# thimabru1010/ResUnet-a_mltsk_keras

Hardware: AMD Instinct MI355X
Metric: training patches/sec (256×256, 6-ch, bs=8/GPU) at 1/2/4/8 MI355X (higher is better)
Workload: dtype bf16; 1 GPU; cfg3: ResUnet-a d6 multitask (seg+bound+dist+color) Tanimoto-dual, 256x256x6, 6 classes, Adam, full train step (fwd+loss+bwd+allreduce+update); global_batch=8, per_gpu_batch=8, parallelism=dp1

## Files before the change

### include/rua_hip.h

```cpp
#ifndef RUA_HIP_H
#define RUA_HIP_H
#include <stdint.h>
#ifdef __cplusplus
extern "C" {
#endif

#define RUA_F32 0
#define RUA_BF16 1
#define RUA_MAX_SEG 6
#define RUA_MAX_BRANCH 4
#define RUA_MAX_WGRAD_BATCH 32
#define RUA_MAX_WGRAD_GROUP 8

#define RUA_OK 0
#define RUA_ERR_ARG (-1)
#define RUA_ERR_LAUNCH (-2)

int rua_version(void);
const char* rua_last_error(void);
int rua_device_info(int* cu_count, int* lds_bytes, char* arch, int arch_len);

typedef struct rua_conv_seg {
  const void* x;
  const void* w;
// ... 91 lines not shown
  const int32_t* overwrite_dev;
} rua_wgrad_desc;
typedef struct rua_wgrad_pending {
  int32_t kind;
  int32_t parts;
  int64_t n;
  const float* partials;
  float* dw;
  int32_t CC;
  int32_t blocks;
  int32_t block_begin, pad;
  const int32_t* overwrite_dev;
} rua_wgrad_pending;
int rua_wgrad_plan(const rua_wgrad_desc* d, rua_wgrad_pending* out);
int rua_wgrad_reduce_batch(const rua_wgrad_pending* items_dev, int n_items, int total_blocks, void* stream);
int rua_conv_wgrad(const rua_wgrad_desc* d, void* stream);
int rua_conv_wgrad_group(const rua_wgrad_desc* d, int n, void* stream);
int rua_wgrad_group_last_grids(void);
int rua_wgrad_group_plan(const rua_wgrad_desc* d, int n, rua_wgrad_pending* out);
int64_t rua_wgrad_workspace_bytes(const rua_wgrad_desc* d);
int rua_wgrad_kind(const rua_wgrad_desc* d);
int rua_wgrad_img_kind(const rua_wgrad_desc* d);

typedef struct rua_wprep_item { int64_t src_off, dst_off; int32_t taps, Cout, C, pad; } rua_wprep_item;
int rua_weight_prep(const float* master, void* w_fwd, void* w_dgrad, const rua_wprep_item* items_dev,
                    int n_items, int max_elems, int dtype, void* stream);
int rua_weight_prep_dgrad(const void* w_fwd, void* w_dgrad, const rua_wprep_item* items_dev, int n_items, int max_elems, const int32_t* blockmap_dev,
                          int n_blocks, int dtype, void* stream);
int rua_wprep_blocks(int taps, int Cout, int C);

// ... 152 lines not shown
int64_t rua_lovasz_workspace_bytes(int64_t M, int C);
int rua_lovasz_grad(const float* p, const float* y, const uint8_t* void_mask, int64_t M, int C, int all_classes, float loss_weight,
                    void* workspace, int64_t workspace_bytes, double* loss_out, float* dp, uint32_t* order_out,
                    rua_lovasz_result* result_dev, void* stream);
int rua_lovasz_dz(int act, const float* p, const float* dp, const float* scale_dev, int64_t M, int C, float* dz, void* stream);

int rua_lr_step(double* state, float* lr_out, int adam, double beta1, double beta2, void* stream);
int rua_adam_step(float* theta, float* g, float* m, float* v, int64_t n, float lr_t, const float* lr_t_dev, float beta1, float beta2,
                  float eps, float grad_scale, int zero_grad, void* stream);
int rua_sgd_step(float* theta, float* g, float* vel, int64_t n, float lr, const float* lr_dev, float momentum, float grad_scale,
                 int zero_grad, void* stream);
int rua_adam_step_w(float* theta, float* g, float* m, float* v, int64_t n, float lr_t, const float* lr_t_dev, float beta1, float beta2,
                    float eps, float grad_scale, int zero_grad, void* wcopy_bf16, void* stream);
int rua_sgd_step_w(float* theta, float* g, float* vel, int64_t n, float lr, const float* lr_dev, float momentum, float grad_scale,
                   int zero_grad, void* wcopy_bf16, void* stream);

#define RUA_OPT_CHUNK 8192
typedef struct rua_opt_chunk { int64_t off; int32_t len; int32_t var; } rua_opt_chunk;
typedef struct rua_opt_var { int32_t chunk_begin, chunk_end, decay, pad; } rua_opt_var;
#define RUA_CLIP_NONE 0
#define RUA_CLIP_GLOBAL_NORM 1
#define RUA_CLIP_NORM 2
#define RUA_CLIP_VALUE 3
int rua_grad_sumsq(const float* g, const rua_opt_chunk* chunks, int n_chunks, double* partials, void* stream);
int rua_clip_finish(const double* partials, int n_chunks, const rua_opt_var* vars, int n_vars, int mode, double c, double grad_scale,
                    int skip_nonfinite, double* var_sumsq, float* coef, int32_t* flag, double* report, void* stream);
int rua_adam_step_seg(float* theta, float* g, float* m, float* v, const rua_opt_chunk* chunks, int n_chunks, const rua_opt_var* vars,
                      const float* coef, const int32_t* flag, const float* lr_dev, const double* lr_state, float beta1, float beta2, float eps,
                      float grad_scale, float clipvalue, double weight_decay, int zero_grad, void* wcopy_bf16, void* stream);
int rua_sgd_step_seg(float* theta, float* g, float* vel, const rua_opt_chunk* chunks, int n_chunks, const rua_opt_var* vars,
// ... 127 lines not shown
```

### resunet_a_mltsk_keras_amd/_lib.py

```python
from __future__ import annotations

import ctypes as C
import os

HERE = os.path.dirname(os.path.abspath(__file__))
LIB_PATH = os.environ.get("RUA_LIB_PATH") or os.path.join(HERE, "librua_hip.so")

RUA_F32, RUA_BF16 = 0, 1
RUA_MAX_SEG, RUA_MAX_BRANCH, RUA_MAX_WGRAD_GROUP, RUA_MAX_WGRAD_BATCH = 6, 4, 8, 32
LOSS_TANIMOTO, LOSS_WCE, LOSS_CE_LOGITS, LOSS_BCE_LOGITS, LOSS_MSE, LOSS_FOCAL_CE, LOSS_FOCAL_BCE = 0, 1, 2, 3, 4, 5, 6
LOSS_LOVASZ, RUA_LOVASZ_MAX_C = 7, 16
ACT_NONE, ACT_SOFTMAX, ACT_SIGMOID = 0, 1, 2

vp, i32, i64, f32, f64 = C.c_void_p, C.c_int32, C.c_int64, C.c_float, C.c_double


class ConvSeg(C.Structure):
    _fields_ = [("x", vp), ("w", vp), ("C", i32), ("Hs", i32), ("Ws", i32), ("up_shift", i32), ("dil", i32), ("taps", i32)]


class ConvDesc(C.Structure):
    _fields_ = [("seg", ConvSeg * RUA_MAX_SEG), ("nseg", i32), ("N", i32), ("H", i32), ("W", i32), ("Cout", i32),
                ("stride", i32), ("dtype", i32), ("bias", vp), ("aux", vp), ("aux_mode", i32), ("mscale", vp),
                ("mshift", vp), ("out_relu", i32), ("accumulate", i32), ("y", vp), ("out_stride", i32), ("OH", i32),
# ... 107 lines not shown
    "rua_wgrad_group_last_grids": ([], i32),
    "rua_wgrad_group_plan": ([C.POINTER(WgradDesc), i32, C.POINTER(WgradPending)], i32),
    "rua_profile_mid_event": ([vp], None),
    "rua_profile_mid_event_fired": ([], i32),
    "rua_prof_event_create": ([], vp),
    "rua_prof_event_record": ([vp, vp], i32),
    "rua_prof_event_elapsed_us": ([vp, vp, C.POINTER(f64)], i32),
    "rua_prof_event_destroy": ([vp], None),
    "rua_graph_kernel_nodes": ([vp, C.POINTER(i32), C.POINTER(i32)], i32),
    "rua_conv_workspace_bytes": ([C.POINTER(ConvDesc)], i64),
    "rua_conv_wgrad": ([C.POINTER(WgradDesc), vp], i32),
    "rua_wgrad_workspace_bytes": ([C.POINTER(WgradDesc)], i64),
    "rua_wgrad_kind": ([C.POINTER(WgradDesc)], i32),
    "rua_wgrad_img_kind": ([C.POINTER(WgradDesc)], i32),
    "rua_wgrad_plan": ([C.POINTER(WgradDesc), C.POINTER(WgradPending)], i32),
    "rua_wgrad_reduce_batch": ([vp, i32, i32, vp], i32),
    "rua_weight_prep": ([vp, vp, vp, vp, i32, i32, i32, vp], i32),
    "rua_weight_prep_dgrad": ([vp, vp, vp, i32, i32, vp, i32, i32, vp], i32),
    "rua_wprep_blocks": ([i32, i32, i32], i32),
    "rua_stem_fwd": ([vp, vp, vp, vp, i64, i32, i32, i32, vp], i32),
    "rua_stem_fwd_stats": ([vp, vp, vp, vp, i64, i32, i32, i32, vp, i32, vp], i32),
    "rua_stem_bwd": ([vp, vp, vp, vp, i64, i32, i32, i32, vp], i32),
    "rua_stem_fwd_pack": ([vp, vp, vp, vp, i64, i32, i32, i32, vp, i32, vp, vp], i32),
    "rua_stem_bwd_fold": ([vp, vp, vp, i32, i32, vp], i32),
    "rua_head_fwd": ([vp, vp, vp, vp, vp, i64, i32, i32, i32, i32, vp], i32),
    "rua_head_fwd_loss": ([vp, vp, vp, vp, vp, vp, vp, vp, i32, i64, i32, i32, i32, i32, vp], i32),
    "rua_head_fwd_loss_rep": ([vp, vp, vp, vp, vp, vp, vp, i32, vp, i32, i64, i32, i32, i32, i32, vp], i32),
    "rua_head_bwd": ([vp, vp, vp, vp, i32, vp, vp, vp, i64, i64, i32, i32, i32, i32, vp], i32),
    "rua_head_bwd_sums": ([vp, vp, vp, vp, i32, vp, vp, vp, vp, i64, i64, i32, i32, i32, i32, vp], i32),
    "rua_col_stats": ([vp, i64, i32, vp, i32, i32, vp], i32),
# ... 28 lines not shown
    "rua_fill_zero": ([vp, i64, vp], i32),
    "rua_tanimoto_sums": ([vp, vp, i32, i64, i32, vp, vp], i32),
    "rua_tanimoto_finalize": ([vp, i32, i64, i32, f32, vp, vp, vp, vp], i32),
    "rua_tanimoto_finalize_rep": ([vp, i32, i32, i64, i32, f32, vp, vp, vp, vp], i32),
    "rua_tanimoto_finalize_multi": ([vp, i32, vp], i32),
    "rua_head_dz_multi": ([vp, i32, vp], i32),
    "rua_tanimoto_ratio": ([vp, i32, i32, vp, vp, vp], i32),
    "rua_pixel_loss": ([i32, vp, vp, vp, vp, i64, i32, vp, vp, vp], i32),
    "rua_head_dz": ([i32, i32, vp, vp, vp, vp, f32, i32, i64, i32, vp, vp], i32),
    "rua_seg_metrics": ([vp, vp, i64, i32, vp, vp], i32),
    "rua_lr_step": ([vp, vp, i32, f64, f64, vp], i32),
    "rua_adam_step": ([vp, vp, vp, vp, i64, f32, vp, f32, f32, f32, f32, i32, vp], i32),
    "rua_sgd_step": ([vp, vp, vp, i64, f32, vp, f32, f32, i32, vp], i32),
    "rua_adam_step_w": ([vp, vp, vp, vp, i64, f32, vp, f32, f32, f32, f32, i32, vp, vp], i32),
    "rua_sgd_step_w": ([vp, vp, vp, i64, f32, vp, f32, f32, i32, vp, vp], i32),
    "rua_grad_sumsq": ([vp, vp, i32, vp, vp], i32),
    "rua_clip_finish": ([vp, i32, vp, i32, i32, f64, f64, i32, vp, vp, vp, vp, vp], i32),
    "rua_adam_step_seg": ([vp, vp, vp, vp, vp, i32, vp, vp, vp, vp, vp, f32, f32, f32, f32, f32, f64, i32, vp, vp], i32),
    "rua_sgd_step_seg": ([vp, vp, vp, vp, i32, vp, vp, vp, vp, vp, f32, f32, f32, f64, i32, vp, vp], i32),
    "rua_state_copy": ([vp, vp, i64, vp, vp], i32),
    "rua_lr_schedule_step": ([vp, vp, LrSchedule, i32, f64, f64, vp], i32),
    "rua_ema_step": ([vp, vp, vp, i64, f32, vp, i32, vp, vp], i32),
    "rua_accum_gate": ([vp, i32, vp, vp], i32),
    "rua_accum_step": ([vp, vp, i64, i32, vp, vp], i32),
    "rua_lr_step_gated": ([vp, vp, i32, f64, f64, vp, vp], i32),
    "rua_lr_schedule_step_gated": ([vp, vp, LrSchedule, i32, f64, f64, vp, vp], i32),
    "rua_grad_sumsq_gated": ([vp, vp, i32, vp, vp, vp], i32),
    "rua_clip_finish_gated": ([vp, i32, vp, i32, i32, f64, f64, i32, vp, vp, vp, vp, vp, vp], i32),
    "rua_lamb_moments": ([vp, vp, vp, vp, vp, i32, vp, vp, vp, vp, f32, f32, f32, f32, f32, f64, vp, vp, vp], i32),
    "rua_lamb_finish": ([vp, vp, i32, vp, i32, vp, vp, vp, vp, vp], i32),
# ... 114 lines not shown
```

### resunet_a_mltsk_keras_amd/csrc/conv_wgrad.hip

```cpp
#include "common.h"

struct WgK {
  const unsigned char* a; const unsigned char* dy; float* dw;
  int C, Hs, Ws, Cout, H, W, N, stride, dil, taps;
  long long M; int pix_per_block, ntc, nti, ksplit;
  int wshift, hshift;
  float* slabs;
  const int* overwrite;
};

template <typename T>
__device__ __forceinline__ void wgrad_kernel_body(const WgK& p, int b) {
  constexpr int VEC = ET<T>::VEC, ES = sizeof(T);
  constexpr int TP = 64;
  constexpr int PPR = 64 / VEC;
  constexpr int ROWB = (ES == 2) ? 192 : 260;
  constexpr int PASS = TP * PPR / 256;
  __shared__ __attribute__((aligned(16))) unsigned char sD[TP * ROWB];
  __shared__ __attribute__((aligned(16))) unsigned char sX[TP * ROWB];

  const int ks = b % p.ksplit; b /= p.ksplit;
  const int ti = b % p.nti; b /= p.nti;
  const int tc = b % p.ntc; b /= p.ntc;
  const int tap = b;
// ... 1848 lines not shown
  return RUA_OK;
}
static int wgrad_issue_alone(const WgLaunch& L, hipStream_t st) {
  const WgLaunch* one = &L;
  const int rc = wgrad_issue(&one, 1, st);
  if (rc != RUA_OK || L.defer || !L.pending.kind) return rc;
  rua_record_mid_event(st);
  return wgrad_reduce(L.pending, st);
}

extern "C" int rua_wgrad_plan(const rua_wgrad_desc* d, rua_wgrad_pending* out) {
  RUA_CHECK_ARG(d && out, "rua_wgrad_plan: null pointer");
  WgLaunch L;
  return wgrad_plan_record(d, 0, &L, out);
}
extern "C" int rua_conv_wgrad(const rua_wgrad_desc* d, void* stream) {
  WgLaunch L;
  const int rc = wgrad_plan_one(d, 0, &L);
  return rc != RUA_OK ? rc : wgrad_issue_alone(L, (hipStream_t)stream);
}

static thread_local int g_wg_group_last_grids = 0;
extern "C" int rua_wgrad_group_last_grids(void) { return g_wg_group_last_grids; }

constexpr int WG_BATCH_MAX_MEMBERS = 4 * RUA_MAX_WGRAD_BATCH;
static bool wgrad_batch_ok(const rua_wgrad_desc* d, int n) {
  if (!(g_tune.wgrad_group & 1) || n > WG_BATCH_MAX_MEMBERS) return false;
  for (int i = 0; i < n; ++i) {
    if (!d[i].a || !d[i].dy || !d[i].dw || d[i].dtype != RUA_BF16 || !d[i].batch || d[i].in_scale) return false;
    if (d[i].C <= 0 || d[i].Cout <= 0 || d[i].C % 8 || d[i].Cout % 8 || (d[i].taps != 1 && d[i].taps != 9)) return false;
// ... 152 lines not shown
```

### resunet_a_mltsk_keras_amd/csrc/loss_optim.hip

```cpp
#include "common.h"

__device__ __forceinline__ void block_atomic_add(double* dst, float v, float* sh , int slot) {
  v = wave_sum(v);
  const int lane = threadIdx.x & 63, wid = threadIdx.x >> 6;
  if (lane == 0) sh[slot * 4 + wid] = v;
  __syncthreads();
  if (threadIdx.x == 0) unsafeAtomicAdd(dst, (double)sh[slot * 4 + 0] + (double)sh[slot * 4 + 1] + (double)sh[slot * 4 + 2] + (double)sh[slot * 4 + 3]);
  __syncthreads();
}

template <bool VM>
__global__ __launch_bounds__(256) void tanimoto_sums_kernel(const float* __restrict__ p, const float* __restrict__ y, long long HW, int C,
                                                            int pix_per_block, double* sums, const uint8_t* __restrict__ vm) {
  __shared__ float sh[4 * 48];
  const int n = blockIdx.y;
  float acc[8][6];
#pragma unroll
  for (int c = 0; c < 8; ++c)
#pragma unroll
    for (int k = 0; k < 6; ++k) acc[c][k] = 0.f;
  long long i = (long long)blockIdx.x * pix_per_block + threadIdx.x;
  long long iend = (long long)(blockIdx.x + 1) * pix_per_block; if (iend > HW) iend = HW;
  for (; i < iend; i += 256) {
    if constexpr (VM) { if (vm[(size_t)n * HW + i]) continue; }
// ... 848 lines not shown
  }
}
template <bool WC>
__global__ __launch_bounds__(256) void sgd_kernel(float* __restrict__ th, float* __restrict__ g, float* __restrict__ vel,
                                                  long long n, float lr, const float* __restrict__ lr_dev, float mu, float gs, int zero, bf16_t* __restrict__ wcopy) {
  if (lr_dev) lr = lr_dev[0];
  for (long long i = (long long)blockIdx.x * 256 + threadIdx.x; i < n; i += (long long)gridDim.x * 256) {
    const float vv = mu * vel[i] - lr * g[i] * gs;
    vel[i] = vv;
    const float tt = th[i] + vv;
    th[i] = tt;
    if (zero) g[i] = 0.f;
    if constexpr (WC) wcopy[i] = (bf16_t)tt;
  }
}
__global__ void lr_step_kernel(double* state, float* lr_out, int adam, double beta1, double beta2, const int32_t* hold) {
  if (blockIdx.x == 0 && threadIdx.x == 0 && !(hold != nullptr && hold[0] != 0)) {
    const double t = state[0] + 1.0;
    state[0] = t;
    double lr = state[1];
    if (adam) lr = lr * sqrt(1.0 - pow(beta2, t)) / (1.0 - pow(beta1, t));
    lr_out[0] = (float)lr;
  }
}
extern "C" int rua_lr_step(double* state, float* lr_out, int adam, double beta1, double beta2, void* stream) {
  RUA_CHECK_ARG(state && lr_out, "rua_lr_step: null pointer");
  hipLaunchKernelGGL(lr_step_kernel, dim3(1), dim3(64), 0, (hipStream_t)stream, state, lr_out, adam, beta1, beta2, (const int32_t*)nullptr);
  RUA_LAUNCH_CHECK("rua_lr_step");
  return RUA_OK;
}
// ... 17 lines not shown
                             float eps, float grad_scale, int zero_grad, void* stream) {
  return rua_adam_step_w(theta, g, m, v, n, lr_t, lr_t_dev, beta1, beta2, eps, grad_scale, zero_grad, nullptr, stream);
}
extern "C" int rua_sgd_step_w(float* theta, float* g, float* vel, int64_t n, float lr, const float* lr_dev, float momentum, float grad_scale,
                              int zero_grad, void* wcopy_bf16, void* stream) {
  RUA_CHECK_ARG(theta && g && vel && n > 0, "rua_sgd_step: bad arguments");
  int64_t gr = (n + 255) / 256; if (gr > 4096) gr = 4096;
  if (wcopy_bf16) hipLaunchKernelGGL((sgd_kernel<true>), dim3((int)gr), dim3(256), 0, (hipStream_t)stream, theta, g, vel, (long long)n, lr, lr_dev, momentum, grad_scale, zero_grad, (bf16_t*)wcopy_bf16);
  else hipLaunchKernelGGL((sgd_kernel<false>), dim3((int)gr), dim3(256), 0, (hipStream_t)stream, theta, g, vel, (long long)n, lr, lr_dev, momentum, grad_scale, zero_grad, (bf16_t*)nullptr);
  RUA_LAUNCH_CHECK("rua_sgd_step");
  return RUA_OK;
}
extern "C" int rua_sgd_step(float* theta, float* g, float* vel, int64_t n, float lr, const float* lr_dev, float momentum, float grad_scale,
                            int zero_grad, void* stream) {
  return rua_sgd_step_w(theta, g, vel, n, lr, lr_dev, momentum, grad_scale, zero_grad, nullptr, stream);
}

__device__ __forceinline__ double wave_sum_f64(double v) {
#pragma unroll
  for (int o = 32; o > 0; o >>= 1) v += __shfl_xor(v, o, 64);
  return v;
}
__global__ __launch_bounds__(256) void grad_sumsq_kernel(const float* __restrict__ g, const rua_opt_chunk* __restrict__ chunks, double* __restrict__ partials,
                                                         const int32_t* __restrict__ hold) {
  __shared__ double sh[4];
  if (hold != nullptr && hold[0] != 0) return;
  const rua_opt_chunk ck = chunks[blockIdx.x];
  const float* gp = g + ck.off;
  const int n4 = ck.len >> 2;
  double acc = 0.0;
// ... 405 lines not shown
```

### resunet_a_mltsk_keras_amd/engine.py

```python
from __future__ import annotations

import contextlib
import ctypes as C
import math
import os
from dataclasses import dataclass, field
from typing import Dict, List, Optional, Tuple

import numpy as np
import torch

from . import _lib as L
from . import accum as AC
from . import clip as CL
from . import lamb as LB
from . import losses as LS
from . import schedules as SC
from .wgrad_queue import WgradQueue, WSpec
from .scenes import (BLEND_MODES, MAP_HEADS, AffineSceneBatch, SceneBatch, blend_table, check_blend_budget, check_photo_table, check_radius,
                     check_scales, check_tolerance, check_views, instance_params, instance_scores, scale_table, sieve_params, sweep_params,
                     view_rows)

BN_EPS, BN_MOMENTUM, KERAS_EPS = 1e-3, 0.99, 1e-7
HEADS = ["seg", "bound", "dist", "color"]
# ... 215 lines not shown
        return self.N * self.H * self.W


def stats_replicas(blocks: int) -> int:
    r = 1
    while r < 32 and r * 8 < blocks:
        r *= 2
    return r


def conv_stats_replicas(blocks: int) -> int:
    r = 1
    while r < 32 and r * 64 < blocks:
        r *= 2
    return r


class Stat:
    __slots__ = ("ptr", "R")

    def __init__(self, ptr, R):
        self.ptr, self.R = ptr, R


class _Dummy:

    def __init__(self, n=0):
        self._n = n

    def data_ptr(self):
# ... 845 lines not shown
                self.wq.one(Bp, WSpec(x, dy, lay["segs"][0]["off"], 1, 1, 9))
                gx, acc = self.gacc(x, masked=x.relu_out)
                sx = None
                if x.bias_offs and x.relu_out and not acc and not self.dry and self.e.bn_dx_bias:
                    sx = self.stat(x.C, (x.M + 127) // 128)
                self.dgrad(Bp, dy, self.Wd(lay["segs"][0]["dst"]), x.C, 1, 9, gx, acc, mask=(x, None, None) if x.relu_out else None, stats2=sx)
                if sx is not None:
                    self.stats_to_grads(Bp, sx, x.C, x.bias_offs)
                    x.bias_done = True
            self.back_steps.append(back)
        return y

    def head(self, x: Ten, cout: int, act: int, hname: str, name=None, lay=None):
        F, tr = self.fwd, self.training
        lay = lay if lay is not None else self.Lconv([x.C], cout, 1, name=name, mfma=False)
        z = self.new(x.N, x.H, x.W, cout, f32=True)
        p = self.new(x.N, x.H, x.W, cout, f32=True)
        y = self.new(x.N, x.H, x.W, cout, f32=True)
        h = dict(name=hname, x=x, z=z, p=p, y=y, lay=lay, act=act, C=cout, slot=len(self.heads))
        sp = self.e.loss
        tani = sp is not None and sp.kind.get(hname) == L.LOSS_TANIMOTO
        if sp is not None and not self.dry and self.e.fuse_head_loss and (tani or hname == "seg"):
            if tani:
                h["sums_rep"] = SUMS_REPLICAS
                h["sums"] = self.salloc((SUMS_REPLICAS + 1) * x.N * cout * 6)
            if hname == "seg":
                h["metrics_done"] = True
            head_args = (x.ptr, self.P(lay["segs"][0]["off"]), self.P(lay["bias"]), z.ptr, p.ptr, y.ptr, h.get("sums"),
                         h.get("sums_rep", 1), self.e.scalars_ptr + 8 * 8 if hname == "seg" else None, x.N, x.H * x.W, x.C, cout, act, self.dt)
            if self.void_ptr is not None:
                F.add("rua_head_fwd_loss_void", *head_args, self.void_ptr)
            else:
                F.add("rua_head_fwd_loss_rep", *head_args)
        else:
            F.add("rua_head_fwd", x.ptr, self.P(lay["segs"][0]["off"]), self.P(lay["bias"]), z.ptr, p.ptr, x.M, x.C, cout, act, self.dt)
        self.heads.append(h)
        return h
# ... 311 lines not shown
class Engine:

    def __init__(self, cfg: ModelConfig, dtype: str = "bf16", device: Optional[torch.device] = None, seed: int = 0,
                 split_k: bool = True, _layout_only: bool = False):
        assert dtype in ("bf16", "f32")
        self.cfg = cfg
        self.dt = L.RUA_BF16 if dtype == "bf16" else L.RUA_F32
        self.dtype = dtype
        self.esize = 2 if dtype == "bf16" else 4
        if cfg.width % 32 != 0:
            raise ValueError(f"width={cfg.width}: the first-stage width must be a multiple of 32 (PSP branches are width/4 "
                             "channels and the MFMA epilogue stores 8-channel pieces)")
        self.dev = None
        self.fuse_bn = os.environ.get("RUA_FUSE_BN", "1") != "0"
        self.fuse_head_loss = os.environ.get("RUA_FUSE_HEAD_LOSS", "1") != "0"
        self.bn_out_stats = os.environ.get("RUA_BN_OUT_STATS", "1") != "0"
        self.bn_dx_bias = os.environ.get("RUA_BN_DX_BIAS", "1") != "0"
        self.pool_pyramid = os.environ.get("RUA_POOL_PYRAMID", "1") != "0"
        self.fold_bn = os.environ.get("RUA_FOLD_BN", "1") != "0"
        self.defer_reduce = os.environ.get("RUA_DEFER_REDUCE", "1") != "0"
        self.flush_bytes = int(float(os.environ.get("RUA_FLUSH_MB", "1e9")) * (1 << 20))
        self.cu_count = 256
        self.split_k = split_k
        self.params = ParamStore()
        self.layers: List[dict] = []
        self.cursor = 0
        self.built = False
        self.loss: Optional[LossSpec] = None
        self.clip: Optional[dict] = None
        self._s_backed = False
# ... 14 lines not shown
        L.lib()
        if not torch.cuda.is_available():
            raise L.RuaError("no HIP device visible: the ResUnet-a training path runs on MI355X only (there is no CPU fallback)")
        self.dev = device or torch.device("cuda", torch.cuda.current_device())
        cu = C.c_int32(0)
        if L.lib().raw("rua_device_info")(C.byref(cu), None, None, 0) == 0 and cu.value > 0:
            self.cu_count = cu.value
        z = lambda n, dt=torch.float32: torch.zeros(max(n, 16), dtype=dt, device=self.dev)
        self.P, self.G, self.M1, self.V1, self.S = z(ps.n), z(ps.n + ps.ns + 16), z(ps.n), z(ps.n), z(ps.ns)
        tdt = torch.bfloat16 if dtype == "bf16" else torch.float32
        self.Wf, self.Wd = z(ps.n, tdt), z(ps.n, tdt)
        self.wgrad_overwrite = os.environ.get("RUA_WGRAD_OVERWRITE", "1") != "0"
        self.ow_flag = torch.zeros(4, dtype=torch.int32, device=self.dev)
        self._ow = 0
        self._g_pending = False
        self.opt_wcopy = dtype == "bf16" and os.environ.get("RUA_OPT_WCOPY", "1") != "0"
        self.wf_fresh = False
        items = np.zeros(0, dtype=[("src", "<i8"), ("dst", "<i8"), ("taps", "<i4"), ("cout", "<i4"), ("c", "<i4"), ("pad", "<i4")])
        rows, mx = [], 1
        for lay in self.layers:
            if "segs" in lay and lay["mfma"]:
                for sg in lay["segs"]:
                    rows.append((sg["off"], sg["dst"], lay["taps"], lay["cout"], sg["C"], 0))
                    mx = max(mx, lay["taps"] * lay["cout"] * sg["C"])
        items = np.array(rows, dtype=items.dtype)
        self.wprep_items = torch.from_numpy(np.frombuffer(items.tobytes(), dtype=np.uint8).copy()).to(self.dev)
        self.wprep_n, self.wprep_max = len(rows), mx
        bm = []
        for i, (_, _, taps, cout, ci, _) in enumerate(rows):
            for b in range(L.lib().raw("rua_wprep_blocks")(taps, cout, ci)):
                bm += [i, 8 * b]
# ... 37 lines not shown
        if not self.built:
            rec = self.params.conv(*args) if kind == "conv" else self.params.bn(*args)
            self.layers.append(rec)
            return rec
        rec = self.layers[self.cursor]
        self.cursor += 1
        return rec

    def graph(self, batch: int, training: bool) -> Graph:
        key = (batch, training)
        if key not in self.graphs:
            assert self.loss is not None, "compile() first"
            self.cursor = 0
            self.graphs[key] = Graph(self, batch, training)
            assert self.cursor == len(self.layers)
        return self.graphs[key]

    def compile(self, spec: LossSpec):
        if self.dev is not None and (self.graphs or self._captured or self._captured_eval or self._captured_dp):
            torch.cuda.synchronize()
        self._captured, self._captured_eval, self._captured_dp = {}, {}, {}
        self._eval_seen = set()
        self._opt_graph = None
        iv = spec.ignore_void
        if iv is not None and (isinstance(iv, bool) or not isinstance(iv, (int, np.integer)) or not 0 <= iv <= 16):
            raise ValueError(f"ignore_void {iv!r}: None (off) or a margin in 0..16")
        CL.check_options(spec.clipnorm, spec.global_clipnorm, spec.clipvalue, spec.weight_decay)
        SC.check_ema_options(spec.use_ema, spec.ema_momentum, spec.ema_overwrite_frequency)
        if spec.lr_schedule is not None and not isinstance(spec.lr_schedule, SC.LearningRateSchedule):
            raise ValueError(f"lr_schedule {spec.lr_schedule!r}: None or a schedule of resunet_a_mltsk_keras_amd.schedules")
        AC.check_steps(spec.gradient_accumulation_steps)
        if spec.optimizer not in ("adam", "sgd", "lamb"):
            raise ValueError(f"optimizer {spec.optimizer!r}: 'adam', 'sgd' or 'lamb'")
        if spec.optimizer == "lamb":
            LB.check_options(spec.beta_1, spec.beta_2, spec.epsilon)
        self._check_loss_options(spec)
        if self._in_ema:
            raise RuntimeError("compile() inside ema_weights(): leave the block first")
        if self.loss is not None and (self.loss.optimizer != spec.optimizer):
            self._t_dev, self._lr_base_dev = -1, None
        self.loss = spec
        self.graphs = {}
        if spec.class_weights is not None:
            self.class_w = torch.tensor(list(spec.class_weights) + [0.0] * 8, dtype=torch.float32, device=self.dev)
            self.class_w_ptr = self.class_w.data_ptr()
        else:
            self.class_w_ptr = None
        self._setup_clip(spec)
        self._sched = SC.to_struct(spec.lr_schedule) if spec.lr_schedule is not None else None
        self.E = None
        if spec.use_ema and self.dev is not None:
            self.E = torch.empty_like(self.P)
            self.reset_ema()
        self.A, self.acc_state = None, None
        self.micro, self._micro_dev = 0, -1
        if spec.gradient_accumulation_steps is not None and self.dev is not None:
            self.A = torch.zeros_like(self.P)
# ... 164 lines not shown
            out[h["name"]] = dict(n_valid=r["n_valid"], n_cls=r["n_cls"], G=r["G"][:Cc], loss_c=r["loss_c"][:Cc], loss=r["loss"], scale=float(r["scale"]))
        return out

    def _backup_state(self, s):
        ck = self.clip
        if ck is not None and ck["s_backup"] is not None:
            L.lib().call("rua_state_copy", ck["s_backup"].data_ptr(), self.S.data_ptr(), self.params.ns, None, C.c_void_p(s))

    def drop_plans(self):
        if self.dev is not None and (self.graphs or self._captured or self._captured_eval or self._captured_dp):
            torch.cuda.synchronize()
        self._captured, self._captured_eval, self._captured_dp = {}, {}, {}
        self._eval_seen = set()
        self._opt_graph = None
        self.graphs = {}
        cu = C.c_int32(0)
        if self.dev is not None and L.lib().raw("rua_device_info")(C.byref(cu), None, None, 0) == 0 and cu.value > 0:
            self.cu_count = cu.value

    def set_weights(self, keras_dict: Dict[str, np.ndarray]):
        P, S = self.params.from_keras(keras_dict)
        self.P.copy_(torch.from_numpy(P)); self.S.copy_(torch.from_numpy(S))
        self.params_changed()

    def params_changed(self):
        self.weights_dirty = True
        self.wf_fresh = False

    def get_weights(self) -> Dict[str, np.ndarray]:
        return self.params.to_keras(self.P.cpu().numpy(), self.S.cpu().numpy())

    def grads_keras(self) -> Dict[str, np.ndarray]:
        return self.params.to_keras(self.G.cpu().numpy())

    def count_params(self) -> int:
        return self.params.count()

    def _stream(self) -> int:
        return torch.cuda.current_stream(self.dev).cuda_stream

    def _prep_weights(self, s):
        if self.weights_dirty:
            if self.opt_wcopy and self.wf_fresh:
                L.lib().call("rua_weight_prep_dgrad", self.Wf.data_ptr(), self.Wd.data_ptr(), self.wprep_items.data_ptr(), self.wprep_n, self.wprep_max,
                             self.wprep_map.data_ptr() if self.wprep_map_n else None, self.wprep_map_n, self.dt, C.c_void_p(s))
            else:
                L.lib().call("rua_weight_prep", self.P.data_ptr(), self.Wf.data_ptr(), self.Wd.data_ptr(), self.wprep_items.data_ptr(),
# ... 152 lines not shown
        sc, w = self.stats_arena[:16], 1
        if self.dist is not None and self.world > 1:
            sc, w = self.dist.reduce_scalars(sc), self.world
        sc = sc.cpu().numpy()
        per = [float(sc[h["slot"]] * h["norm"] / w) for h in g.heads]
        total = sum(self.loss.weight[h["name"]] * v for h, v in zip(g.heads, per))
        M = g.outputs["seg"]["x"].M * w
        if g.void_u8 is not None:
            M = float(sc[9] + sc[10] + sc[11] + sc[12]) / g.outputs["seg"]["C"]
        mets = [float(sc[8] / M) if M > 0 else 0.0, float(sc[9]), float(sc[10]), float(sc[11]), float(sc[12])]
        if self.cfg.multitasking:
            return [total] + per + mets
        return [total] + mets

    def _set_overwrite(self, v: int):
        if self._ow != v:
            self.ow_flag.fill_(v)
            self._ow = v

    def forward_backward(self, x=None, y=None, _whole_step: bool = False, norm_type: Optional[int] = None, void_mask=None, photo=None):
        self._check_scene(x, y, norm_type)
        self._check_void(x, norm_type, void_mask)
        photo = self._check_photo(x, norm_type, photo)
        self._set_overwrite(1 if (_whole_step and self.wgrad_overwrite and not self._g_pending) else 0)
        if not _whole_step:
            self._g_pending = True
        B = x.shape[0] if x is not None else self._last_B
        self._last_B = B
        g = self.graph(B, True)
        s = self._stream()
# ... 82 lines not shown
            flag = ck["flag"].data_ptr() if ck["skip"] else None
            if sp.optimizer == "lamb":
                self._launch_lamb(flag, grad_scale, wc, sv)
            elif sp.optimizer == "adam":
                lib.call("rua_adam_step_seg", self.P.data_ptr(), self.G.data_ptr(), self.M1.data_ptr(), self.V1.data_ptr(), ck["chunks"].data_ptr(),
                         ck["n_chunks"], ck["vars"].data_ptr(), ck["coef"].data_ptr(), flag, self.lr_dev.data_ptr(), self.lr_state.data_ptr(),
                         sp.beta_1, sp.beta_2, KERAS_EPS, grad_scale, ck["cv"], ck["wd"], 1, wc, sv)
            else:
                lib.call("rua_sgd_step_seg", self.P.data_ptr(), self.G.data_ptr(), self.M1.data_ptr(), ck["chunks"].data_ptr(), ck["n_chunks"],
                         ck["vars"].data_ptr(), ck["coef"].data_ptr(), flag, self.lr_dev.data_ptr(), self.lr_state.data_ptr(), sp.momentum,
                         grad_scale, ck["cv"], ck["wd"], 1, wc, sv)
            self._launch_ema(wc, flag, s)
            if ck["s_backup"] is not None:
                lib.call("rua_state_copy", self.S.data_ptr(), ck["s_backup"].data_ptr(), self.params.ns, flag, sv)
            return
        if sp.optimizer == "adam":
            L.lib().call("rua_adam_step_w", self.P.data_ptr(), self.G.data_ptr(), self.M1.data_ptr(), self.V1.data_ptr(), self.params.n,
                         0.0, self.lr_dev.data_ptr(), sp.beta_1, sp.beta_2, KERAS_EPS, grad_scale, 1, wc, C.c_void_p(s))
        else:
            L.lib().call("rua_sgd_step_w", self.P.data_ptr(), self.G.data_ptr(), self.M1.data_ptr(), self.params.n, 0.0,
                         self.lr_dev.data_ptr(), sp.momentum, grad_scale, 1, wc, C.c_void_p(s))
        self._launch_ema(wc, None, s)

    def _launch_optimizer_accum(self, grad_scale, s):
        sp, ck, lib, sv = self.loss, self.clip, L.lib(), C.c_void_p(s)
        k, adam = int(sp.gradient_accumulation_steps), 1 if sp.optimizer == "adam" else 0
        hold = self.acc_state.data_ptr() + 4
        flag = ck["flag"].data_ptr()
        both = flag + 4
        wc = self.Wf.data_ptr() if self.opt_wcopy else None
        lib.call("rua_accum_gate", self.acc_state.data_ptr(), k, hold, sv)
# ... 17 lines not shown
                     grad_scale, ck["cv"], ck["wd"], 1, wc, sv)
        self._launch_ema(wc, both, s)
        if ck["s_backup"] is not None:
            lib.call("rua_state_copy", self.S.data_ptr(), ck["s_backup"].data_ptr(), self.params.ns, flag, sv)

    def _launch_ema(self, wc, flag, s):
        if self.E is None:
            return
        sp = self.loss
        L.lib().call("rua_ema_step", self.E.data_ptr(), self.P.data_ptr(), wc, self.params.n, float(sp.ema_momentum), self.lr_state.data_ptr(),
                     int(sp.ema_overwrite_frequency or 0), flag, C.c_void_p(s))

    def optimizer_step(self, grad_scale: float = 1.0):
        self._set_lr()
        self._launch_optimizer(grad_scale, self._stream())
        self.weights_dirty = True
        self._g_pending = False
        self._s_backed = False

    def _issue_step(self, g: Graph):
        s = self._stream()
        self._zero_arena(g, s)
        self._backup_state(s)
        self.weights_dirty = True
        self._prep_weights(s)
        g.fwd.run(s)
        g.loss_plan.run(s)
        g.bwd.run(s)
        self._launch_optimizer(1.0, s)

    def _graph_step(self, x, y, norm_type: Optional[int] = None, void_mask=None, photo=None):
        B = x.shape[0] if x is not None else self._last_B
        self._last_B = B
        g = self.graph(B, True)
        self._put_batch(g, x, y, norm_type, void_mask=void_mask, photo=photo)
        self._set_lr()
        self._set_overwrite(1 if (self.wgrad_overwrite and not self._g_pending) else 0)
        self._g_pending = False
        cap = self._captured.get(B)
        if cap is None:
            self._issue_step(g)
            torch.cuda.synchronize()
            cap = torch.cuda.CUDAGraph()
            with torch.cuda.graph(cap):
                self._issue_step(g)
            self._captured[B] = cap
            self.weights_dirty = True
            return g
        self._ensure_forward_copy()
        cap.replay()
        self.weights_dirty = True
        return g

# ... 51 lines not shown
                import sys
                print(f"[resunet_a] HIP-graph capture of the data-parallel step failed ({exc}); running it eagerly", file=sys.stderr, flush=True)
                torch.cuda.synchronize()
                ok = 0
            if self.dist.all_ranks_ok(ok) == 0:
                self.dp_graph = False
                self.weights_dirty = True
                return g
            self._captured_dp[B] = pieces
            self._opt_graph = opt
            self.weights_dirty = True
            return g
        self._set_lr()
        self._set_overwrite(1 if (self.wgrad_overwrite and not self._g_pending) else 0)
        self._g_pending = False
        self._ensure_forward_copy()
        red.begin()
        for pi, (cap, buckets) in enumerate(pieces):
            cap.replay()
            if self.dp_fence:
                self._dp_fence.zero_()
            elif os.environ.get("RUA_DP_SYNC") == "1":
                torch.cuda.synchronize()
            if pi == 0:
                self.dist.start_state_reduce(self)
            for b in buckets:
                red.ready(b)
        self.dist.reduce_gradients(self)
        self._opt_graph.replay()
        self.weights_dirty = True
# ... 293 lines not shown
```

### resunet_a_mltsk_keras_amd/wgrad_queue.py

```python
import ctypes as C
from collections import namedtuple
from typing import List

import torch

from . import _lib as L

WS_TAIL_BYTES = 264 << 10


WSpec = namedtuple("WSpec", "a dy dw_off stride dil taps in_bn", defaults=(None,))


def chunks(items: List, n: int) -> List[List]:
    return [items[i:i + n] for i in range(0, len(items), n)]


class WgradQueue:

    def __init__(self, e, bwd, dt: int, dry: bool, alloc, keep, G, issue):
        self.e, self.bwd, self.dt, self.dry, self.alloc, self.keep, self.G, self.issue = e, bwd, dt, dry, alloc, keep, G, issue
        self.pending: List[tuple] = []
        self.pending_bytes = 0
        self.pending_bucket = 0
        self.later: List[tuple] = []

    def desc(self, sp: WSpec, group: int = 0):
        d = L.WgradDesc()
        d.group_members = group
        d.a, d.C, d.Hs, d.Ws = sp.a.ptr, sp.a.C, sp.a.H, sp.a.W
        if sp.in_bn is not None:
            d.in_scale, d.in_shift, d.in_relu = sp.in_bn.scale, sp.in_bn.shift, 1
        d.dy, d.Cout, d.H, d.W = sp.dy.ptr, sp.dy.C, sp.dy.H, sp.dy.W
        d.N, d.stride, d.dil, d.taps, d.dtype = sp.dy.N, sp.stride, sp.dil, sp.taps, self.dt
        d.dw, d.grads = self.G(sp.dw_off), (sp.dw_off,)
        if not self.dry:
            if self.e.wgrad_overwrite:
                d.overwrite_dev = self.e.ow_flag.data_ptr()
            d.workspace, d.workspace_bytes = self.e.scratch.data_ptr(), self.e.scratch.numel() * 4
        return d
# ... 113 lines not shown
            self.pending.append((rec, o))

    def flush(self):
        self.issue_later()
        self.pending_bytes = 0
        if not self.pending:
            return
        blocks = 0
        for r, _ in self.pending:
            r.block_begin = blocks
            blocks += r.blocks
        recs = (L.WgradPending * len(self.pending))(*[r for r, _ in self.pending])
        table = torch.frombuffer(bytearray(bytes(recs)), dtype=torch.uint8).to(self.e.dev)
        self.keep(table)
        self.bwd.add("rua_wgrad_reduce_batch", table.data_ptr(), len(self.pending), blocks, grads=[off for _, off in self.pending])
        self.pending = []
```

Measured before the change: 1353 patches/s.

## Skip optimizer gradient zeroing for wgrad-overwritten params and drop dead tanimoto logits

Adds a per-64-float4 bitmap, built when the graph is recorded, marking gradient ranges that a single wgrad kernel fully overwrites each step. New Adam and SGD kernels consult this bitmap together with the overwrite flag and skip writing zeros to those gradient slices. The full buffer is re-zeroed lazily when the overwrite mode is turned off or gradients are read. Separately, fused Tanimoto heads in training no longer allocate or compute the logits tensor, which is now rebuilt on demand. This trims memory writes in the optimizer and forward pass, at the cost of fairly involved bookkeeping where a wrong bitmap could leave stale gradients.

```diff
diff --git a/include/rua_hip.h b/include/rua_hip.h
--- a/include/rua_hip.h
+++ b/include/rua_hip.h
@@ -129,6 +129,7 @@
 } rua_wgrad_pending;
 int rua_wgrad_plan(const rua_wgrad_desc* d, rua_wgrad_pending* out);
 int rua_wgrad_reduce_batch(const rua_wgrad_pending* items_dev, int n_items, int total_blocks, void* stream);
+int rua_wgrad_stores_dw(const rua_wgrad_desc* d);
 int rua_conv_wgrad(const rua_wgrad_desc* d, void* stream);
 int rua_conv_wgrad_group(const rua_wgrad_desc* d, int n, void* stream);
 int rua_wgrad_group_last_grids(void);
@@ -311,6 +312,10 @@
                     float eps, float grad_scale, int zero_grad, void* wcopy_bf16, void* stream);
 int rua_sgd_step_w(float* theta, float* g, float* vel, int64_t n, float lr, const float* lr_dev, float momentum, float grad_scale,
                    int zero_grad, void* wcopy_bf16, void* stream);
+int rua_adam_step_wz(float* theta, float* g, float* m, float* v, int64_t n, float lr_t, const float* lr_t_dev, float beta1, float beta2,
+                     float eps, float grad_scale, int zero_grad, void* wcopy_bf16, const uint64_t* zero_bits, const int32_t* overwrite_dev, void* stream);
+int rua_sgd_step_wz(float* theta, float* g, float* vel, int64_t n, float lr, const float* lr_dev, float momentum, float grad_scale,
+                    int zero_grad, void* wcopy_bf16, const uint64_t* zero_bits, const int32_t* overwrite_dev, void* stream);
 
 #define RUA_OPT_CHUNK 8192
 typedef struct rua_opt_chunk { int64_t off; int32_t len; int32_t var; } rua_opt_chunk;
diff --git a/resunet_a_mltsk_keras_amd/_lib.py b/resunet_a_mltsk_keras_amd/_lib.py
--- a/resunet_a_mltsk_keras_amd/_lib.py
+++ b/resunet_a_mltsk_keras_amd/_lib.py
@@ -145,6 +145,7 @@
     "rua_wgrad_kind": ([C.POINTER(WgradDesc)], i32),
     "rua_wgrad_img_kind": ([C.POINTER(WgradDesc)], i32),
     "rua_wgrad_plan": ([C.POINTER(WgradDesc), C.POINTER(WgradPending)], i32),
+    "rua_wgrad_stores_dw": ([C.POINTER(WgradDesc)], i32),
     "rua_wgrad_reduce_batch": ([vp, i32, i32, vp], i32),
     "rua_weight_prep": ([vp, vp, vp, vp, i32, i32, i32, vp], i32),
     "rua_weight_prep_dgrad": ([vp, vp, vp, i32, i32, vp, i32, i32, vp], i32),
@@ -203,6 +204,8 @@
     "rua_sgd_step": ([vp, vp, vp, i64, f32, vp, f32, f32, i32, vp], i32),
     "rua_adam_step_w": ([vp, vp, vp, vp, i64, f32, vp, f32, f32, f32, f32, i32, vp, vp], i32),
     "rua_sgd_step_w": ([vp, vp, vp, i64, f32, vp, f32, f32, i32, vp, vp], i32),
+    "rua_adam_step_wz": ([vp, vp, vp, vp, i64, f32, vp, f32, f32, f32, f32, i32, vp, vp, vp, vp], i32),
+    "rua_sgd_step_wz": ([vp, vp, vp, i64, f32, vp, f32, f32, i32, vp, vp, vp, vp], i32),
     "rua_grad_sumsq": ([vp, vp, i32, vp, vp], i32),
     "rua_clip_finish": ([vp, i32, vp, i32, i32, f64, f64, i32, vp, vp, vp, vp, vp], i32),
     "rua_adam_step_seg": ([vp, vp, vp, vp, vp, i32, vp, vp, vp, vp, vp, f32, f32, f32, f32, f32, f64, i32, vp, vp], i32),
diff --git a/resunet_a_mltsk_keras_amd/csrc/conv_wgrad.hip b/resunet_a_mltsk_keras_amd/csrc/conv_wgrad.hip
--- a/resunet_a_mltsk_keras_amd/csrc/conv_wgrad.hip
+++ b/resunet_a_mltsk_keras_amd/csrc/conv_wgrad.hip
@@ -1886,6 +1886,22 @@
   WgLaunch L;
   return wgrad_plan_record(d, 0, &L, out);
 }
+extern "C" int rua_wgrad_stores_dw(const rua_wgrad_desc* d) {
+  if (!d || !d->overwrite_dev) return 0;
+  WgLaunch L;
+  if (wgrad_plan_one(d, 0, &L) != RUA_OK) return 0;
+  if (L.pending.kind) return L.defer ? 1 : 0;
+  if (WG_KERNEL[L.kernel].args != WG_ARGS_K) return 0;
+  if (L.kernel == WG_IMGS8 || L.kernel == WG_IMGS16) return 1;
+  const WgK& k = L.k.g;
+  if (!k.overwrite || k.ksplit != 1) return 0;
+  if (d->batch && d->dtype == RUA_BF16) {
+    const long long ndw = (long long)d->taps * d->Cout * d->C;
+    const int cap = (g_tune.wgrad_slabs && ndw % 4 == 0) ? slab_capacity(d, ndw) : 0;
+    return (cap >= 2 && L.defer) || (k.M + 63) / 64 == 1 ? 1 : 0;
+  }
+  return 1;
+}
 extern "C" int rua_conv_wgrad(const rua_wgrad_desc* d, void* stream) {
   WgLaunch L;
   const int rc = wgrad_plan_one(d, 0, &L);
diff --git a/resunet_a_mltsk_keras_amd/csrc/loss_optim.hip b/resunet_a_mltsk_keras_amd/csrc/loss_optim.hip
--- a/resunet_a_mltsk_keras_amd/csrc/loss_optim.hip
+++ b/resunet_a_mltsk_keras_amd/csrc/loss_optim.hip
@@ -886,6 +886,74 @@
     if constexpr (WC) wcopy[i] = (bf16_t)tt;
   }
 }
+template <bool WC>
+__global__ __launch_bounds__(256) void adam_kernel_wz(float* __restrict__ th, float* __restrict__ g, float* __restrict__ m, float* __restrict__ v,
+                                                      long long n, float lr_t, const float* __restrict__ lr_dev, float b1, float b2, float eps, float gs,
+                                                      int zero, const unsigned long long* __restrict__ zbits, const int* __restrict__ ow, bf16_t* __restrict__ wcopy) {
+  if (lr_dev) lr_t = lr_dev[0];
+  const bool all = ow[0] == 0;
+  const long long n4 = n >> 2;
+  auto upd = [&](float gg_, float& mm, float& vv, float& tt) {
+    const float gg = gg_ * gs;
+    mm = b1 * mm + (1.f - b1) * gg;
+    vv = b2 * vv + (1.f - b2) * gg * gg;
+    tt -= lr_t * mm / (sqrtf(vv) + eps);
+  };
+  const int wave = __builtin_amdgcn_readfirstlane((int)(threadIdx.x >> 6)), lane = (int)(threadIdx.x & 63);
+  for (long long w = (long long)blockIdx.x * 4 + wave; (w << 6) < n4; w += (long long)gridDim.x * 4) {
+    const unsigned long long bits = !zero ? 0ull : all ? ~0ull : zbits[w];
+    const long long i = (w << 6) + lane;
+    if (i >= n4) continue;
+    const float4 g4 = reinterpret_cast<const float4*>(g)[i];
+    float4 m4 = reinterpret_cast<float4*>(m)[i], v4 = reinterpret_cast<float4*>(v)[i], t4 = reinterpret_cast<float4*>(th)[i];
+    upd(g4.x, m4.x, v4.x, t4.x); upd(g4.y, m4.y, v4.y, t4.y); upd(g4.z, m4.z, v4.z, t4.z); upd(g4.w, m4.w, v4.w, t4.w);
+    reinterpret_cast<float4*>(m)[i] = m4; reinterpret_cast<float4*>(v)[i] = v4; reinterpret_cast<float4*>(th)[i] = t4;
+    if ((bits >> lane) & 1ull) reinterpret_cast<float4*>(g)[i] = make_float4(0.f, 0.f, 0.f, 0.f);
+    if constexpr (WC) reinterpret_cast<uint2*>(wcopy)[i] = make_uint2(ET<bf16_t>::pk(t4.x, t4.y), ET<bf16_t>::pk(t4.z, t4.w));
+  }
+  for (long long i = (n4 << 2) + (long long)blockIdx.x * 256 + threadIdx.x; i < n; i += (long long)gridDim.x * 256) {
+    float mm = m[i], vv = v[i], tt = th[i];
+    upd(g[i], mm, vv, tt);
+    m[i] = mm; v[i] = vv; th[i] = tt;
+    if (zero) g[i] = 0.f;
+    if constexpr (WC) wcopy[i] = (bf16_t)tt;
+  }
+}
+template <bool WC>
+__global__ __launch_bounds__(256) void sgd_kernel_wz(float* __restrict__ th, float* __restrict__ g, float* __restrict__ vel, long long n, float lr,
+                                                     const float* __restrict__ lr_dev, float mu, float gs, int zero, const unsigned long long* __restrict__ zbits,
+                                                     const int* __restrict__ ow, bf16_t* __restrict__ wcopy) {
+  if (lr_dev) lr = lr_dev[0];
+  const bool all = ow[0] == 0;
+  const long long n4 = n >> 2;
+  auto upd = [&](float gg, float& vv_, float& tt_) {
+#pragma clang fp contract(off)
+    const float t = (lr * gg) * gs;
+    float vv;
+    if constexpr (WC) vv = __builtin_fmaf(mu, vv_, -t); else vv = mu * vv_ - t;
+    vv_ = vv;
+    tt_ = tt_ + vv;
+  };
+  const int wave = __builtin_amdgcn_readfirstlane((int)(threadIdx.x >> 6)), lane = (int)(threadIdx.x & 63);
+  for (long long w = (long long)blockIdx.x * 4 + wave; (w << 6) < n4; w += (long long)gridDim.x * 4) {
+    const unsigned long long bits = !zero ? 0ull : all ? ~0ull : zbits[w];
+    const long long i = (w << 6) + lane;
+    if (i >= n4) continue;
+    const float4 g4 = reinterpret_cast<const float4*>(g)[i];
+    float4 v4 = reinterpret_cast<float4*>(vel)[i], t4 = reinterpret_cast<float4*>(th)[i];
+    upd(g4.x, v4.x, t4.x); upd(g4.y, v4.y, t4.y); upd(g4.z, v4.z, t4.z); upd(g4.w, v4.w, t4.w);
+    reinterpret_cast<float4*>(vel)[i] = v4; reinterpret_cast<float4*>(th)[i] = t4;
+    if ((bits >> lane) & 1ull) reinterpret_cast<float4*>(g)[i] = make_float4(0.f, 0.f, 0.f, 0.f);
+    if constexpr (WC) reinterpret_cast<uint2*>(wcopy)[i] = make_uint2(ET<bf16_t>::pk(t4.x, t4.y), ET<bf16_t>::pk(t4.z, t4.w));
+  }
+  for (long long i = (n4 << 2) + (long long)blockIdx.x * 256 + threadIdx.x; i < n; i += (long long)gridDim.x * 256) {
+    float vv = vel[i], tt = th[i];
+    upd(g[i], vv, tt);
+    vel[i] = vv; th[i] = tt;
+    if (zero) g[i] = 0.f;
+    if constexpr (WC) wcopy[i] = (bf16_t)tt;
+  }
+}
 __global__ void lr_step_kernel(double* state, float* lr_out, int adam, double beta1, double beta2, const int32_t* hold) {
   if (blockIdx.x == 0 && threadIdx.x == 0 && !(hold != nullptr && hold[0] != 0)) {
     const double t = state[0] + 1.0;
@@ -933,6 +1001,32 @@
 extern "C" int rua_sgd_step(float* theta, float* g, float* vel, int64_t n, float lr, const float* lr_dev, float momentum, float grad_scale,
                             int zero_grad, void* stream) {
   return rua_sgd_step_w(theta, g, vel, n, lr, lr_dev, momentum, grad_scale, zero_grad, nullptr, stream);
+}
+extern "C" int rua_adam_step_wz(float* theta, float* g, float* m, float* v, int64_t n, float lr_t, const float* lr_t_dev, float beta1, float beta2,
+                                float eps, float grad_scale, int zero_grad, void* wcopy_bf16, const uint64_t* zero_bits, const int32_t* overwrite_dev, void* stream) {
+  RUA_CHECK_ARG(theta && g && m && v && n > 0, "rua_adam_step_wz: bad arguments");
+  RUA_CHECK_ARG(zero_bits && overwrite_dev, "rua_adam_step_wz: the zero bitmap and the overwrite flag are required (rua_adam_step_w zeroes everything)");
+  RUA_CHECK_ARG((((size_t)theta | (size_t)g | (size_t)m | (size_t)v) & 15) == 0 && ((size_t)wcopy_bf16 & 7) == 0 && ((size_t)zero_bits & 7) == 0 &&
+                ((size_t)overwrite_dev & 3) == 0, "rua_adam_step_wz: buffers must be 16-byte aligned (bitmap: 8, flag: 4)");
+  int64_t gr = (n / 4 + 255) / 256; if (gr > 4096) gr = 4096; if (gr < 1) gr = 1;
+  const unsigned long long* zb = reinterpret_cast<const unsigned long long*>(zero_bits);
+  if (wcopy_bf16) hipLaunchKernelGGL((adam_kernel_wz<true>), dim3((int)gr), dim3(256), 0, (hipStream_t)stream, theta, g, m, v, (long long)n, lr_t, lr_t_dev, beta1, beta2, eps, grad_scale, zero_grad, zb, (const int*)overwrite_dev, (bf16_t*)wcopy_bf16);
+  else hipLaunchKernelGGL((adam_kernel_wz<false>), dim3((int)gr), dim3(256), 0, (hipStream_t)stream, theta, g, m, v, (long long)n, lr_t, lr_t_dev, beta1, beta2, eps, grad_scale, zero_grad, zb, (const int*)overwrite_dev, (bf16_t*)nullptr);
+  RUA_LAUNCH_CHECK("rua_adam_step_wz");
+  return RUA_OK;
+}
+extern "C" int rua_sgd_step_wz(float* theta, float* g, float* vel, int64_t n, float lr, const float* lr_dev, float momentum, float grad_scale,
+                               int zero_grad, void* wcopy_bf16, const uint64_t* zero_bits, const int32_t* overwrite_dev, void* stream) {
+  RUA_CHECK_ARG(theta && g && vel && n > 0, "rua_sgd_step_wz: bad arguments");
+  RUA_CHECK_ARG(zero_bits && overwrite_dev, "rua_sgd_step_wz: the zero bitmap and the overwrite flag are required (rua_sgd_step_w zeroes everything)");
+  RUA_CHECK_ARG((((size_t)theta | (size_t)g | (size_t)vel) & 15) == 0 && ((size_t)wcopy_bf16 & 7) == 0 && ((size_t)zero_bits & 7) == 0 &&
+                ((size_t)overwrite_dev & 3) == 0, "rua_sgd_step_wz: buffers must be 16-byte aligned (bitmap: 8, flag: 4)");
+  int64_t gr = (n / 4 + 255) / 256; if (gr > 4096) gr = 4096; if (gr < 1) gr = 1;
+  const unsigned long long* zb = reinterpret_cast<const unsigned long long*>(zero_bits);
+  if (wcopy_bf16) hipLaunchKernelGGL((sgd_kernel_wz<true>), dim3((int)gr), dim3(256), 0, (hipStream_t)stream, theta, g, vel, (long long)n, lr, lr_dev, momentum, grad_scale, zero_grad, zb, (const int*)overwrite_dev, (bf16_t*)wcopy_bf16);
+  else hipLaunchKernelGGL((sgd_kernel_wz<false>), dim3((int)gr), dim3(256), 0, (hipStream_t)stream, theta, g, vel, (long long)n, lr, lr_dev, momentum, grad_scale, zero_grad, zb, (const int*)overwrite_dev, (bf16_t*)nullptr);
+  RUA_LAUNCH_CHECK("rua_sgd_step_wz");
+  return RUA_OK;
 }
 
 __device__ __forceinline__ double wave_sum_f64(double v) {
diff --git a/resunet_a_mltsk_keras_amd/engine.py b/resunet_a_mltsk_keras_amd/engine.py
--- a/resunet_a_mltsk_keras_amd/engine.py
+++ b/resunet_a_mltsk_keras_amd/engine.py
@@ -253,6 +253,23 @@
     while r < 32 and r * 64 < blocks:
         r *= 2
     return r
+
+
+class LazyLogits:
+    ptr = None
+
+    def __init__(self, g: "Graph", h: dict):
+        self.g, self.h = g, h
+
+    @property
+    def t(self) -> torch.Tensor:
+        g, h = self.g, self.h
+        x, lay = h["x"], h["lay"]
+        z = torch.empty((x.N, x.H, x.W, h["C"]), dtype=torch.float32, device=g.dev)
+        p = torch.empty_like(z)
+        L.lib().call("rua_head_fwd", x.ptr, g.P(lay["segs"][0]["off"]), g.P(lay["bias"]), z.data_ptr(), p.data_ptr(), x.M, x.C, h["C"], h["act"], g.dt,
+                     C.c_void_p(g.e._stream()))
+        return z
 
 
 class Stat:
@@ -1128,13 +1145,17 @@
     def head(self, x: Ten, cout: int, act: int, hname: str, name=None, lay=None):
         F, tr = self.fwd, self.training
         lay = lay if lay is not None else self.Lconv([x.C], cout, 1, name=name, mfma=False)
-        z = self.new(x.N, x.H, x.W, cout, f32=True)
+        sp = self.e.loss
+        tani = sp is not None and sp.kind.get(hname) == L.LOSS_TANIMOTO
+        fused = sp is not None and not self.dry and self.e.fuse_head_loss and (tani or hname == "seg")
+        dead_z = fused and tani and tr and self.e.drop_dead_logits
+        z = None if dead_z else self.new(x.N, x.H, x.W, cout, f32=True)
         p = self.new(x.N, x.H, x.W, cout, f32=True)
         y = self.new(x.N, x.H, x.W, cout, f32=True)
         h = dict(name=hname, x=x, z=z, p=p, y=y, lay=lay, act=act, C=cout, slot=len(self.heads))
-        sp = self.e.loss
-        tani = sp is not None and sp.kind.get(hname) == L.LOSS_TANIMOTO
-        if sp is not None and not self.dry and self.e.fuse_head_loss and (tani or hname == "seg"):
+        if dead_z:
+            h["z"] = z = LazyLogits(self, h)
+        if fused:
             if tani:
                 h["sums_rep"] = SUMS_REPLICAS
                 h["sums"] = self.salloc((SUMS_REPLICAS + 1) * x.N * cout * 6)
@@ -1476,6 +1497,7 @@
         self.dev = None
         self.fuse_bn = os.environ.get("RUA_FUSE_BN", "1") != "0"
         self.fuse_head_loss = os.environ.get("RUA_FUSE_HEAD_LOSS", "1") != "0"
+        self.drop_dead_logits = os.environ.get("RUA_DROP_DEAD_LOGITS", "1") != "0"
         self.bn_out_stats = os.environ.get("RUA_BN_OUT_STATS", "1") != "0"
         self.bn_dx_bias = os.environ.get("RUA_BN_DX_BIAS", "1") != "0"
         self.pool_pyramid = os.environ.get("RUA_POOL_PYRAMID", "1") != "0"
@@ -1520,7 +1542,12 @@
         self.ow_flag = torch.zeros(4, dtype=torch.int32, device=self.dev)
         self._ow = 0
         self._g_pending = False
-        self.opt_wcopy = dtype == "bf16" and os.environ.get("RUA_OPT_WCOPY", "1") != "0"
+        self.opt_zero_map = os.environ.get("RUA_OPT_ZERO_MAP", "1") != "0"
+        self._zero_sets: Dict[int, np.ndarray] = {}
+        self._zero_host = np.full((ps.n // 4 + 63) // 64 + 1, np.uint64(0xFFFFFFFFFFFFFFFF), dtype=np.uint64)
+        self.zero_bits = torch.from_numpy(self._zero_host.view(np.int64).copy()).to(self.dev)
+        self._g_stale = False
+        self.opt_wcopy =dtype == "bf16" and os.environ.get("RUA_OPT_WCOPY", "1") != "0"
         self.wf_fresh = False
         items = np.zeros(0, dtype=[("src", "<i8"), ("dst", "<i8"), ("taps", "<i4"), ("cout", "<i4"), ("c", "<i4"), ("pad", "<i4")])
         rows, mx = [], 1
@@ -1588,7 +1615,87 @@
             self.cursor = 0
             self.graphs[key] = Graph(self, batch, training)
             assert self.cursor == len(self.layers)
+            if training:
+                self._record_zero_map(self.graphs[key])
         return self.graphs[key]
+
+    def _record_zero_map(self, g: Graph):
+        if not self.opt_zero_map:
+            return
+        lib, n, base = L.lib(), self.params.n, self.G.data_ptr()
+        cand: Dict[int, list] = {}
+        others: List[int] = []
+        for plan in (g.fwd, g.loss_plan, g.bwd):
+            for _, name, args, grads in plan.calls:
+                if name == "rua_wgrad_reduce_batch":
+                    continue
+                if name not in ("rua_conv_wgrad", "rua_conv_wgrad_group"):
+                    others += list(grads)
+                    continue
+                descs = [args[0]._obj] if name == "rua_conv_wgrad" else [args[0][i] for i in range(args[1])]
+                offs = []
+                for d in descs:
+                    off = (d.dw - base) // 4
+                    offs.append(off)
+                    c = cand.setdefault(off, [d.taps * d.Cout * d.C, 0, True, True])
+                    c[1] += 1
+                    c[2] = c[2] and c[0] == d.taps * d.Cout * d.C and bool(d.overwrite_dev) and lib.raw("rua_wgrad_stores_dw")(C.byref(d)) == 1
+                    c[3] = c[3] and bool(d.defer)
+                others += [o for o in grads if o not in offs]
+        reduces: Dict[int, int] = {}
+        for off, kind in g.wq.reduced:
+            if kind in (1, 2) and off in cand:
+                reduces[off] = reduces.get(off, 0) + 1
+            else:
+                others.append(off)
+        keep = np.zeros(n // 4, dtype=bool)
+        others_a = np.array(sorted(set(others)), dtype=np.int64)
+        for off, (nel, nd, stores, deferred) in cand.items():
+            r = reduces.get(off, 0)
+            hit = np.searchsorted(others_a, off + nel) - np.searchsorted(others_a, off)
+            if nd == 1 and stores and r <= 1 and (r == 0 or deferred) and hit == 0 and off >= 0 and off % 4 == 0 and off + nel <= n:
+                keep[off // 4:(off + nel) // 4] = True
+        words = np.full(self._zero_host.size, np.uint64(0xFFFFFFFFFFFFFFFF), dtype=np.uint64)
+        packed = np.packbits(~keep, bitorder="little")
+        as_bytes = words.view(np.uint8)
+        full = keep.size // 8
+        as_bytes[:full] = packed[:full]
+        if keep.size % 8:
+            as_bytes[full] = packed[full] | np.uint8((0xFF << (keep.size % 8)) & 0xFF)
+        self._zero_sets[g.B] = words
+        self._upload_zero_map()
+
+    def _upload_zero_map(self):
+        union = np.full(self._zero_host.size, np.uint64(0xFFFFFFFFFFFFFFFF), dtype=np.uint64)
+        if self._zero_sets:
+            union = np.bitwise_or.reduce(np.stack(list(self._zero_sets.values())), axis=0)
+        if not np.array_equal(union, self._zero_host):
+            self._flush_stale()
+            self._zero_host = union
+            self.zero_bits.copy_(torch.from_numpy(union.view(np.int64).copy()))
+
+    def _reset_zero_map(self):
+        if self.dev is None:
+            return
+        self._zero_sets = {}
+        self._upload_zero_map()
+
+    def unzeroed_ranges(self) -> List[Tuple[int, int]]:
+        bits = np.unpackbits(self._zero_host.view(np.uint8), bitorder="little")[:self.params.n // 4]
+        edge = np.flatnonzero(np.diff(np.concatenate(([1], bits, [1]))))
+        return [(int(a) * 4, int(b - a) * 4) for a, b in zip(edge[0::2], edge[1::2])]
+
+    def _flush_stale(self):
+        if self._g_stale:
+            self.G[:self.params.n].zero_()
+            self._g_stale = False
+
+    def _uses_zero_map(self) -> bool:
+        return self.opt_zero_map and self.A is None and self.clip is None and self.loss.optimizer in ("adam", "sgd")
+
+    def _after_optimizer(self):
+        if self._uses_zero_map() and self._ow == 1:
+            self._g_stale = True
 
     def compile(self, spec: LossSpec):
         if self.dev is not None and (self.graphs or self._captured or self._captured_eval or self._captured_dp):
@@ -1615,6 +1722,7 @@
             self._t_dev, self._lr_base_dev = -1, None
         self.loss = spec
         self.graphs = {}
+        self._reset_zero_map()
         if spec.class_weights is not None:
             self.class_w = torch.tensor(list(spec.class_weights) + [0.0] * 8, dtype=torch.float32, device=self.dev)
             self.class_w_ptr = self.class_w.data_ptr()
@@ -1809,6 +1917,7 @@
         self._eval_seen = set()
         self._opt_graph = None
         self.graphs = {}
+        self._reset_zero_map()
         cu = C.c_int32(0)
         if self.dev is not None and L.lib().raw("rua_device_info")(C.byref(cu), None, None, 0) == 0 and cu.value > 0:
             self.cu_count = cu.value
@@ -1826,6 +1935,7 @@
         return self.params.to_keras(self.P.cpu().numpy(), self.S.cpu().numpy())
 
     def grads_keras(self) -> Dict[str, np.ndarray]:
+        self._flush_stale()
         return self.params.to_keras(self.G.cpu().numpy())
 
     def count_params(self) -> int:
@@ -2008,6 +2118,8 @@
         return [total] + mets
 
     def _set_overwrite(self, v: int):
+        if v == 0:
+            self._flush_stale()
         if self._ow != v:
             self.ow_flag.fill_(v)
             self._ow = v
@@ -2120,7 +2232,15 @@
             if ck["s_backup"] is not None:
                 lib.call("rua_state_copy", self.S.data_ptr(), ck["s_backup"].data_ptr(), self.params.ns, flag, sv)
             return
-        if sp.optimizer == "adam":
+        if self._uses_zero_map():
+            zb, ow = self.zero_bits.data_ptr(), self.ow_flag.data_ptr()
+            if sp.optimizer == "adam":
+                L.lib().call("rua_adam_step_wz", self.P.data_ptr(), self.G.data_ptr(), self.M1.data_ptr(), self.V1.data_ptr(), self.params.n,
+                             0.0, self.lr_dev.data_ptr(), sp.beta_1, sp.beta_2, KERAS_EPS, grad_scale, 1, wc, zb, ow, C.c_void_p(s))
+            else:
+                L.lib().call("rua_sgd_step_wz", self.P.data_ptr(), self.G.data_ptr(), self.M1.data_ptr(), self.params.n, 0.0,
+                             self.lr_dev.data_ptr(), sp.momentum, grad_scale, 1, wc, zb, ow, C.c_void_p(s))
+        elif sp.optimizer == "adam":
             L.lib().call("rua_adam_step_w", self.P.data_ptr(), self.G.data_ptr(), self.M1.data_ptr(), self.V1.data_ptr(), self.params.n,
                          0.0, self.lr_dev.data_ptr(), sp.beta_1, sp.beta_2, KERAS_EPS, grad_scale, 1, wc, C.c_void_p(s))
         else:
@@ -2168,6 +2288,7 @@
     def optimizer_step(self, grad_scale: float = 1.0):
         self._set_lr()
         self._launch_optimizer(grad_scale, self._stream())
+        self._after_optimizer()
         self.weights_dirty = True
         self._g_pending = False
         self._s_backed = False
@@ -2191,6 +2312,7 @@
         self._set_lr()
         self._set_overwrite(1 if (self.wgrad_overwrite and not self._g_pending) else 0)
         self._g_pending = False
+        self._after_optimizer()
         cap = self._captured.get(B)
         if cap is None:
             self._issue_step(g)
@@ -2272,6 +2394,7 @@
         self._set_lr()
         self._set_overwrite(1 if (self.wgrad_overwrite and not self._g_pending) else 0)
         self._g_pending = False
+        self._after_optimizer()
         self._ensure_forward_copy()
         red.begin()
         for pi, (cap, buckets) in enumerate(pieces):
diff --git a/resunet_a_mltsk_keras_amd/wgrad_queue.py b/resunet_a_mltsk_keras_amd/wgrad_queue.py
--- a/resunet_a_mltsk_keras_amd/wgrad_queue.py
+++ b/resunet_a_mltsk_keras_amd/wgrad_queue.py
@@ -24,6 +24,7 @@
         self.pending_bytes = 0
         self.pending_bucket = 0
         self.later: List[tuple] = []
+        self.reduced: List[tuple] = []
 
     def desc(self, sp: WSpec, group: int = 0):
         d = L.WgradDesc()
@@ -167,4 +168,5 @@
         table = torch.frombuffer(bytearray(bytes(recs)), dtype=torch.uint8).to(self.e.dev)
         self.keep(table)
         self.bwd.add("rua_wgrad_reduce_batch", table.data_ptr(), len(self.pending), blocks, grads=[off for _, off in self.pending])
+        self.reduced += [(off, int(r.kind)) for r, off in self.pending]
         self.pending = []
```

Measured after the change: 1363 patches/s (median of 6 runs). No clear change (+0.7%).
